# thetengda/OKVIS2-X

Hardware: AMD Instinct MI355X
Metric: Gauss-Newton iters/sec on 50-KF/2000-landmark window; ATE vs CPU ref (higher is better)
Workload: dtype f64; 1 GPU; 2048 independent S50 windows (50 KF / 2000 landmarks / 16000 reprojections, 49 IMU factors), DENSE_SCHUR + DOGLEG, all tolerances 0; windows_total=2048, windows_per_gpu=2048, parallelism=replicas x1 (one window batch per GPU, no collective in the loop)

## Files before the change

okvis2-x_amd/csrc/chol_tiles.hpp:

```cpp
#pragma once
#include "dev_clock.hpp"
#include "device_problem.hpp"
#include "okvisgpu_math.hpp"

namespace okg {

constexpr int kLd = kTile + 1;


typedef double dbl4 __attribute__((ext_vector_type(4)));

__device__ __forceinline__ bool cholSelect(const DevProblem& P, int w) {
  const WinState& s = P.st[w];
  return !s.done && s.need_gn && !s.gn_failed;
}

__device__ __forceinline__ int tileBlocks(const DevProblem& P, int w, int k) {
  const int fdim = P.win_fdim[w], g0 = P.win_sgap[2 * w], gl = P.win_sgap[2 * w + 1];
  int end = min(fdim - kTile * k, kTile);
  if (gl > 0 && g0 >= kTile * k && g0 < kTile * (k + 1)) end = min(end, g0 - kTile * k);
  return max(1, (end + 15) >> 4);
}

struct TileSrc {
  const double* S;
  const double* W;
  const int16_t* fu;
  int T;
  int64_t ld;
  __device__ __forceinline__ const double* at(int i, int j, int k) const {
    return (gmem(fu)[i * T + j] < k ? W : S) + (int64_t)i * kTile * ld + j * kTile;
  }
};
__device__ __forceinline__ TileSrc tileSrc(const DevProblem& P, int w, int64_t ld) {
  return TileSrc{P.S + P.win_soff[w], P.W + P.win_soff[w], P.tile_fu + P.win_tnzoff[w], (int)(ld / kTile), ld};
}

__device__ __forceinline__ void loadTile(const double* A, int64_t ld, int r0, int c0, double* s, int t) {
  double2 v[8];
#pragma unroll
  for (int u = 0; u < 8; ++u) {
    const int e = t + 256 * u, r = e >> 5, c = 2 * (e & 31);
    v[u] = *gmem(reinterpret_cast<const double2*>(A + (int64_t)(r0 + r) * ld + c0 + c));
  }
#pragma unroll
  for (int u = 0; u < 8; ++u) {
    const int e = t + 256 * u, r = e >> 5, c = 2 * (e & 31);
    s[r * kLd + c] = v[u].x;
    s[r * kLd + c + 1] = v[u].y;
  }
}

__device__ __forceinline__ void mfmaTileNT(const double* sA, const double* sB, dbl4 acc[2][2], int t) {
  const int wave = t >> 6, lane = t & 63;
  const int r0 = 32 * (wave >> 1), c0 = 32 * (wave & 1);
  const int lr = lane & 15, lk = lane >> 4;
#pragma unroll
  for (int a = 0; a < 2; ++a)
#pragma unroll
    for (int b = 0; b < 2; ++b) acc[a][b] = dbl4{0.0, 0.0, 0.0, 0.0};
#pragma unroll 4
  for (int kk = 0; kk < kTile; kk += 4) {
    double av[2], bv[2];
#pragma unroll
    for (int a = 0; a < 2; ++a) av[a] = sA[(r0 + 16 * a + lr) * kLd + kk + lk];
#pragma unroll
    for (int b = 0; b < 2; ++b) bv[b] = sB[(c0 + 16 * b + lr) * kLd + kk + lk];
#pragma unroll
    for (int a = 0; a < 2; ++a)
#pragma unroll
      for (int b = 0; b < 2; ++b) acc[a][b] = __builtin_amdgcn_mfma_f64_16x16x4f64(av[a], bv[b], acc[a][b], 0, 0, 0);
  }
}

template <bool SUB>
__device__ __forceinline__ void storeTile(double* A, int64_t ld, int r0g, int c0g, const dbl4 acc[2][2], int t) {
  const int wave = t >> 6, lane = t & 63;
  const int r0 = 32 * (wave >> 1), c0 = 32 * (wave & 1);
#pragma unroll
  for (int a = 0; a < 2; ++a)
#pragma unroll
    for (int b = 0; b < 2; ++b)
#pragma unroll
      for (int reg = 0; reg < 4; ++reg) {
        const int rr = r0 + 16 * a + (lane >> 4) + 4 * reg;
        const int cc = c0 + 16 * b + (lane & 15);
        auto dst = gmemw(A + (int64_t)(r0g + rr) * ld + c0g + cc);
        if (SUB) *dst -= acc[a][b][reg];
        else *dst = acc[a][b][reg];
      }
}

__device__ __forceinline__ void loadC(const double* A, int64_t ld, dbl4 c[2][2], int t) {
  const int wave = t >> 6, lane = t & 63;
  const int r0 = 32 * (wave >> 1), c0 = 32 * (wave & 1);
#pragma unroll
  for (int a = 0; a < 2; ++a)
#pragma unroll
    for (int b = 0; b < 2; ++b)
#pragma unroll
      for (int reg = 0; reg < 4; ++reg)
        c[a][b][reg] = gmem(A)[(int64_t)(r0 + 16 * a + (lane >> 4) + 4 * reg) * ld + c0 + 16 * b + (lane & 15)];
}
__device__ __forceinline__ void storeTileSub(double* A, int64_t ld, const dbl4 c[2][2], const dbl4 acc[2][2], int t) {
  const int wave = t >> 6, lane = t & 63;
  const int r0 = 32 * (wave >> 1), c0 = 32 * (wave & 1);
#pragma unroll
  for (int a = 0; a < 2; ++a)
#pragma unroll
    for (int b = 0; b < 2; ++b)
#pragma unroll
      for (int reg = 0; reg < 4; ++reg)
        gmemw(A)[(int64_t)(r0 + 16 * a + (lane >> 4) + 4 * reg) * ld + c0 + 16 * b + (lane & 15)] = c[a][b][reg] - acc[a][b][reg];
}

__device__ __forceinline__ double rsqrtRefined(double d) {
  double r = __builtin_amdgcn_rsq(d);
  const double h = 0.5 * d;
  r = r * (1.5 - h * r * r);
  r = r * (1.5 - h * r * r);
  return r;
}

template <int KB>
__device__ __forceinline__ void mfma16(const double* a, int lda, const double* b, int ldbk, int ldbn, double sign,
                                       dbl4& acc, int lane) {
  const int lr = lane & 15, lk = lane >> 4;
#pragma unroll
  for (int q = 0; q < 4 * KB; ++q) {
    const double av = sign * a[lr * lda + 4 * q + lk];
    const double bv = b[(4 * q + lk) * ldbk + lr * ldbn];
    acc = __builtin_amdgcn_mfma_f64_16x16x4f64(av, bv, acc, 0, 0, 0);
  }
}
__device__ __forceinline__ dbl4 loadC16(const double* c, int ldc, int lane) {
  dbl4 v;
#pragma unroll
  for (int r = 0; r < 4; ++r) v[r] = c[((lane >> 4) + 4 * r) * ldc + (lane & 15)];
  return v;
}
__device__ __forceinline__ void storeC16(double* c, int ldc, const dbl4& v, int lane) {
#pragma unroll
  for (int r = 0; r < 4; ++r) c[((lane >> 4) + 4 * r) * ldc + (lane & 15)] = v[r];
}

__device__ __forceinline__ int ldsAcquire(int* p) {
  return __hip_atomic_load(p, __ATOMIC_ACQUIRE, __HIP_MEMORY_SCOPE_WORKGROUP);
}
__device__ __forceinline__ void ldsRelease(int* p, int v) {
  __hip_atomic_store(p, v, __ATOMIC_RELEASE, __HIP_MEMORY_SCOPE_WORKGROUP);
}
__device__ __forceinline__ int ldsAcquireL(int* p) {
  const int v = __hip_atomic_load(p, __ATOMIC_RELAXED, __HIP_MEMORY_SCOPE_WORKGROUP);
  __builtin_amdgcn_fence(__ATOMIC_ACQUIRE, "workgroup", "local");
  return v;
}
__device__ __forceinline__ void ldsReleaseL(int* p, int v) {
  __builtin_amdgcn_fence(__ATOMIC_RELEASE, "workgroup", "local");
  __hip_atomic_store(p, v, __ATOMIC_RELAXED, __HIP_MEMORY_SCOPE_WORKGROUP);
}
#ifndef OKG_WAIT_SLEEP
#define OKG_WAIT_SLEEP 1
#endif
template <bool LOCAL = false>
__device__ __forceinline__ bool waitFlag(int* p, int v, int* fail) {
  for (;;) {
    if ((LOCAL ? ldsAcquireL(p) : ldsAcquire(p)) >= v) return true;
    if (LOCAL ? ldsAcquireL(fail) : ldsAcquire(fail)) return false;
    __builtin_amdgcn_s_sleep(OKG_WAIT_SLEEP);
  }
}
template <bool LOCAL = false>
__device__ __forceinline__ void waveBarrier(int* ctr, int& gen, int n, int lane) {
  ++gen;
  if (LOCAL) {
    __builtin_amdgcn_fence(__ATOMIC_RELEASE, "workgroup", "local");
    if (lane == 0) __hip_atomic_fetch_add(ctr, 1, __ATOMIC_RELAXED, __HIP_MEMORY_SCOPE_WORKGROUP);
    while (ldsAcquireL(ctr) < gen * n) __builtin_amdgcn_s_sleep(OKG_WAIT_SLEEP);
  } else {
    if (lane == 0) __hip_atomic_fetch_add(ctr, 1, __ATOMIC_RELEASE, __HIP_MEMORY_SCOPE_WORKGROUP);
    while (ldsAcquire(ctr) < gen * n) __builtin_amdgcn_s_sleep(OKG_WAIT_SLEEP);
  }
}

__device__ __forceinline__ bool chol8Row(const double* sA, int c0, double (&r)[8], double (&x)[8], double (&rl)[8]) {
  double D[8][8];
#pragma unroll
  for (int m = 0; m < 8; ++m)
#pragma unroll
    for (int k = 0; k <= m; ++k) D[m][k] = sA[(c0 + m) * kLd + c0 + k];
  bool bad = false;
#pragma unroll
  for (int c = 0; c < 8; ++c) {
    const double d = D[c][c];
    if (!(d > 0.0)) bad = true;
    rl[c] = rsqrtRefined(d);
#pragma unroll
    for (int m = c + 1; m < 8; ++m) D[m][c] *= rl[c];
    x[c] = r[c] * rl[c];
#pragma unroll
    for (int m = c + 1; m < 8; ++m) {
      D[m][m] -= D[m][c] * D[m][c];
      r[m] -= x[c] * D[m][c];
    }
#pragma unroll
    for (int m = c + 2; m < 8; ++m)
#pragma unroll
      for (int k = c + 1; k < m; ++k) D[m][k] -= D[m][c] * D[k][c];
  }
  return !bad;
}
__device__ __forceinline__ void storeRow8(double* sA, int c0, const double (&x)[8], int i) {
  if (i >= c0) {
#pragma unroll
    for (int k = 0; k < 8; ++k)
      if (i >= c0 + 8 || k <= i - c0) sA[i * kLd + c0 + k] = x[k];
  }
}
__device__ __forceinline__ void inv8(const double* sA, const double* sRl, double* xd, int c0, int lane) {
  if (lane >= 8) return;
  double L[8][8], rl[8];
#pragma unroll
  for (int m = 0; m < 8; ++m) {
    rl[m] = sRl[c0 + m];
#pragma unroll
    for (int k = 0; k < m; ++k) L[m][k] = sA[(c0 + m) * kLd + c0 + k];
  }
  double y[8];
#pragma unroll
  for (int m = 0; m < 8; ++m) {
    double v = (m == lane) ? 1.0 : 0.0;
#pragma unroll
    for (int k = 0; k < m; ++k) v -= L[m][k] * y[k];
    y[m] = v * rl[m];
  }
#pragma unroll
  for (int m = 0; m < 8; ++m) xd[m * kLd + lane] = y[m];
}
__device__ __forceinline__ bool subPanel8(double* sA, double* xd, double* sRl, int c0, int lane) {
  double r[8], x[8], rl[8];
#pragma unroll
  for (int k = 0; k < 8; ++k) r[k] = sA[lane * kLd + c0 + k];
  if (!chol8Row(sA, c0, r, x, rl)) return false;
  storeRow8(sA, c0, x, lane);
  if (lane == 0) {
#pragma unroll
    for (int k = 0; k < 8; ++k) sRl[c0 + k] = rl[k];
  }
  __builtin_amdgcn_wave_barrier();
  inv8(sA, sRl, xd, c0, lane);
  return true;
}

__device__ __forceinline__ void trailingFrom(double* sA, int c0, int cs, int wg, int nw, int lane) {
  const int cb0 = cs >> 4;
  const bool part = (cs & 15) != 0;
  const int lr = lane & 15, lk = lane >> 4;
  int idx = 0;
  for (int rb = cb0; rb < 4; ++rb)
    for (int cb = cb0; cb <= rb; ++cb, ++idx) {
      if (idx % nw != wg) continue;
      double* C = sA + 16 * rb * kLd + 16 * cb;
      dbl4 acc = loadC16(C, kLd, lane);
#pragma unroll
      for (int q = 0; q < 2; ++q) {
        const double av = -sA[(16 * rb + lr) * kLd + c0 + 4 * q + lk];
        const double bv = sA[(16 * cb + lr) * kLd + c0 + 4 * q + lk];
        acc = __builtin_amdgcn_mfma_f64_16x16x4f64(av, bv, acc, 0, 0, 0);
      }
      if (part && cb == cb0 && lr < 8) continue;
#pragma unroll
      for (int r = 0; r < 4; ++r)
        if (!(part && rb == cb0 && r < 2)) C[(lk + 4 * r) * kLd + lr] = acc[r];
    }
}
__device__ __forceinline__ void trailing8(double* sA, int c0, int wg, int nw, int lane) {
  trailingFrom(sA, c0, c0 + 8, wg, nw, lane);
}

__device__ __forceinline__ void xDiag16(const double* sA, double* sX, int q, int lane) {
  const int m = lane >> 3, j = lane & 7;
  const int b = 16 * q;
  double t = 0.0;
#pragma unroll
  for (int k = 0; k < 8; ++k) t += sA[(b + 8 + m) * kLd + b + k] * sX[(b + k) * kLd + b + j];
  sX[(b + 8 + m) * kLd + b + j] = t;
  __builtin_amdgcn_wave_barrier();
  double tk[8];
#pragma unroll
  for (int k = 0; k < 8; ++k) tk[k] = sX[(b + 8 + k) * kLd + b + j];
  double v = 0.0;
#pragma unroll
  for (int k = 0; k < 8; ++k) v += sX[(b + 8 + m) * kLd + b + 8 + k] * tk[k];
  __builtin_amdgcn_wave_barrier();
  sX[(b + 8 + m) * kLd + b + j] = -v;
}
__device__ __forceinline__ void xOffDiag16(const double* sA, double* sX, int q, int j, int lane) {
  dbl4 acc = dbl4{0.0, 0.0, 0.0, 0.0};
  for (int m = j; m < q; ++m)
    mfma16<1>(sA + 16 * q * kLd + 16 * m, kLd, sX + 16 * m * kLd + 16 * j, kLd, 1, 1.0, acc, lane);
  double* Xqj = sX + 16 * q * kLd + 16 * j;
  storeC16(Xqj, kLd, acc, lane);
  dbl4 x = dbl4{0.0, 0.0, 0.0, 0.0};
  mfma16<1>(sX + 16 * q * kLd + 16 * q, kLd, Xqj, kLd, 1, -1.0, x, lane);
  storeC16(Xqj, kLd, x, lane);
}
__device__ __forceinline__ void yBlock16(const double* sX, double* sy, int q, int lane) {
  const int r = 16 * q + (lane & 15), p = lane >> 4;
  double xv[16], rv[16];
#pragma unroll
  for (int it = 0; it < 16; ++it) {
    xv[it] = sX[r * kLd + p + 4 * it];
    rv[it] = sy[p + 4 * it];
  }
  double a = 0.0;
#pragma unroll
  for (int it = 0; it < 16; ++it) a += (p + 4 * it <= r) ? xv[it] * rv[it] : 0.0;
  a += __shfl_xor(a, 16, 64);
  a += __shfl_xor(a, 32, 64);
  if (p == 0) sy[kTile + r] = a;
}
__host__ __device__ constexpr bool persistentCaller(int kCaller) { return kCaller >= 10; }
template <int kCaller>
__device__ __forceinline__ void xStoreRows16(const double* sX, double* Li, int q, int g, int lane) {
  double2 v[3];
#pragma unroll
  for (int it = 0; it < 3; ++it) {
    const int e = min(64 * g + lane + 192 * it, 511), r = 16 * q + (e >> 5), c = 2 * (e & 31);
    v[it] = double2{(c <= r) ? sX[r * kLd + c] : 0.0, (c + 1 <= r) ? sX[r * kLd + c + 1] : 0.0};
  }
#pragma unroll
  for (int it = 0; it < 3; ++it) {
    const int e = 64 * g + lane + 192 * it, r = 16 * q + (e >> 5), c = 2 * (e & 31);
    if (e < 512 && (!persistentCaller(kCaller) || c <= r)) *gmemw(reinterpret_cast<double2*>(Li + r * kTile + c)) = v[it];
  }
}

__host__ __device__ constexpr bool teamCaller(int kCaller) { return kCaller >= 20; }
constexpr int kPotrfBarriers = 3;
template <int kCaller>
__device__ __forceinline__ void potrfSync(int* sFl, int& tgen, int lane) {
  if (teamCaller(kCaller)) waveBarrier<true>(&sFl[4], tgen, 4, lane);
  else ldsBarrier();
}
template <int kCaller>
__device__ __forceinline__ bool potrfTileBody(const double* Sg, int64_t ld, double* Li, double* workk, double* sA, double* sX,
                                              double* sy, double* sRl, int* sFl, int t, bool haveTile, int tgen0, int nq) {
  const int wave = t >> 6, lane = t & 63;
  int tgen = tgen0;
  CLK_INIT
  if (!haveTile) loadTile(Sg, ld, 0, 0, sA, t);
  nq = __builtin_amdgcn_readfirstlane(nq);
#pragma unroll
  for (int u = 0; u < 16; ++u) {
    const int e = t + 256 * u;
    sX[(e >> 6) * kLd + (e & 63)] = 0.0;
  }
  if (t < 4) sFl[t] = 0;
  potrfSync<kCaller>(sFl, tgen, lane);
  CLK(4)
  if (wave == 0) {
    const int i = lane;
    if (i >= 16 * nq) {
      sX[i * kLd + i] = 1.0;
      sy[kTile + i] = sy[i];
    }
    double xp[8];
#pragma unroll
    for (int k = 0; k < 8; ++k) xp[k] = 0.0;
#pragma unroll 1
    for (int s = 0; s < 2 * nq; ++s) {
      const int c0 = 8 * s;
      CLK(25)
      if (s >= 2 && !waitFlag<true>(&sFl[1], s - 1, &sFl[2])) break;
      CLK(21)
      double r[8], x[8], rl[8];
#pragma unroll
      for (int k = 0; k < 8; ++k) r[k] = sA[i * kLd + c0 + k];
      if (s >= 1) {
#pragma unroll
        for (int hb = 0; hb < 2; ++hb) {
          double Lq[4][8];
#pragma unroll
          for (int c = 0; c < 4; ++c)
#pragma unroll
            for (int m = 0; m < 8; ++m) Lq[c][m] = sA[(c0 + m) * kLd + c0 - 8 + 4 * hb + c];
#pragma unroll
          for (int c = 0; c < 4; ++c)
#pragma unroll
            for (int m = 0; m < 8; ++m) r[m] -= xp[4 * hb + c] * Lq[c][m];
        }
        asm volatile("" ::"v"(r[0]), "v"(r[1]), "v"(r[2]), "v"(r[3]), "v"(r[4]), "v"(r[5]), "v"(r[6]), "v"(r[7]));
        if (i >= c0) {
#pragma unroll
          for (int k = 0; k < 8; ++k) sA[i * kLd + c0 + k] = r[k];
        }
        __builtin_amdgcn_wave_barrier();
      }
      CLK(22)
      if (!chol8Row(sA, c0, r, x, rl)) {
        if (lane == 0) ldsReleaseL(&sFl[2], 1);
        break;
      }
      asm volatile("" ::"v"(x[7]));
      CLK(23)
      if (i >= c0) {
#pragma unroll
        for (int k = 0; k < 8; ++k) sA[i * kLd + c0 + k] = x[k];
      }
      if (lane == 0) {
#pragma unroll
        for (int k = 0; k < 8; ++k) sRl[c0 + k] = rl[k];
        ldsReleaseL(&sFl[0], s + 1);
      }
      CLK(24)
#pragma unroll
      for (int k = 0; k < 8; ++k) xp[k] = x[k];
    }
  } else {
    const int g = wave - 1;
    int gen = 0;
#pragma unroll 1
    for (int s = 0; s < 2 * nq; ++s) {
      if (!waitFlag<true>(&sFl[0], s + 1, &sFl[2])) break;
      if (g == 0) inv8(sA, sRl, sX + 8 * s * kLd + 8 * s, 8 * s, lane);
      if (s < 6) trailingFrom(sA, 8 * s, 8 * s + 16, g, 3, lane);
      waveBarrier<true>(&sFl[3], gen, 3, lane);
      if (g == 0 && lane == 0) ldsReleaseL(&sFl[1], s + 1);
      if (s & 1) {
        const int q = s >> 1;
        if (g == 0) xDiag16(sA, sX, q, lane);
        waveBarrier<true>(&sFl[3], gen, 3, lane);
        if (g < q) xOffDiag16(sA, sX, q, g, lane);
        waveBarrier<true>(&sFl[3], gen, 3, lane);
        if (g == 0) yBlock16(sX, sy, q, lane);
        for (int qs = q, qe = q + 1 < nq ? q + 1 : 4; qs < qe; ++qs) xStoreRows16<kCaller>(sX, Li, qs, g, lane);
      }
    }
  }
  potrfSync<kCaller>(sFl, tgen, lane);
  CLK(5)
  if (sFl[2]) return false;
  if (t < kTile) {
    const double y = sy[kTile + t];
    sy[t] = y;
    if (!persistentCaller(kCaller)) gmemw(workk)[t] = y;
  }
  potrfSync<kCaller>(sFl, tgen, lane);
  CLK(10)
  return true;
}
template <int kCaller>
__device__ __noinline__ bool potrfTile(const double* Sg, int64_t ld, double* Li, double* workk, double* sA, double* sX, double* sy,
                                      double* sRl, int* sFl, int t, bool haveTile, int tgen0 = 0, int nq = 4) {
  return potrfTileBody<kCaller>(Sg, ld, Li, workk, sA, sX, sy, sRl, sFl, t, haveTile, tgen0, nq);
}

__device__ __forceinline__ void accToLds(double* s, const dbl4 acc[2][2], int t) {
  const int wave = t >> 6, lane = t & 63;
  const int r0 = 32 * (wave >> 1), c0 = 32 * (wave & 1);
#pragma unroll
  for (int a = 0; a < 2; ++a)
#pragma unroll
    for (int b = 0; b < 2; ++b)
#pragma unroll
      for (int reg = 0; reg < 4; ++reg) s[(r0 + 16 * a + (lane >> 4) + 4 * reg) * kLd + c0 + 16 * b + (lane & 15)] = acc[a][b][reg];
}
__device__ __forceinline__ void accSubToLds(double* s, const dbl4 c[2][2], const dbl4 acc[2][2], int t) {
  const int wave = t >> 6, lane = t & 63;
  const int r0 = 32 * (wave >> 1), c0 = 32 * (wave & 1);
#pragma unroll
  for (int a = 0; a < 2; ++a)
#pragma unroll
    for (int b = 0; b < 2; ++b)
#pragma unroll
      for (int reg = 0; reg < 4; ++reg)
        s[(r0 + 16 * a + (lane >> 4) + 4 * reg) * kLd + c0 + 16 * b + (lane & 15)] = c[a][b][reg] - acc[a][b][reg];
}

__device__ __forceinline__ void mfmaPanelRows(const double* sA, const double* sX, dbl4 acc[4], int t) {
  const int wave = t >> 6, lane = t & 63;
  const int lr = lane & 15, lk = lane >> 4;
#pragma unroll
  for (int cb = 0; cb < 4; ++cb) acc[cb] = dbl4{0.0, 0.0, 0.0, 0.0};
#pragma unroll
  for (int kk = 0; kk < kTile; kk += 4) {
    const double av = sA[(16 * wave + lr) * kLd + kk + lk];
#pragma unroll
    for (int cb = kk >> 4; cb < 4; ++cb)
      acc[cb] = __builtin_amdgcn_mfma_f64_16x16x4f64(av, sX[(16 * cb + lr) * kLd + kk + lk], acc[cb], 0, 0, 0);
  }
}
__device__ __forceinline__ void storePanelRows(double* A, int64_t ld, const dbl4 acc[4], int t) {
  const int wave = t >> 6, lane = t & 63;
#pragma unroll
  for (int cb = 0; cb < 4; ++cb)
#pragma unroll
    for (int reg = 0; reg < 4; ++reg)
      gmemw(A)[(int64_t)(16 * wave + (lane >> 4) + 4 * reg) * ld + 16 * cb + (lane & 15)] = acc[cb][reg];
}
__device__ __forceinline__ void panelRowsToLds(double* s, const dbl4 acc[4], int t) {
  const int wave = t >> 6, lane = t & 63;
#pragma unroll
  for (int cb = 0; cb < 4; ++cb)
#pragma unroll
    for (int reg = 0; reg < 4; ++reg) s[(16 * wave + (lane >> 4) + 4 * reg) * kLd + 16 * cb + (lane & 15)] = acc[cb][reg];
}
__device__ __forceinline__ int diagRb(int wave, int e) { return wave == 0 ? (e == 0 ? 0 : 1) : (wave == 1 ? 2 : 3); }
__device__ __forceinline__ int diagCb(int wave, int e) { return wave == 0 ? (e == 0 ? 0 : e - 1) : (wave == 3 ? 2 + e : e); }
__device__ __forceinline__ int diagN(int wave) { return wave < 2 ? 3 : 2; }
__device__ __forceinline__ void mfmaDiagNT(const double* sL, dbl4 acc[3], int t) {
  const int wave = t >> 6, lane = t & 63;
  const int lr = lane & 15, lk = lane >> 4;
  const int n = diagN(wave);
  int ra[3], rb[3];
#pragma unroll
  for (int e = 0; e < 3; ++e) {
    ra[e] = (16 * diagRb(wave, e) + lr) * kLd + lk;
    rb[e] = (16 * diagCb(wave, e) + lr) * kLd + lk;
    acc[e] = dbl4{0.0, 0.0, 0.0, 0.0};
  }
#pragma unroll 4
  for (int kk = 0; kk < kTile; kk += 4) {
#pragma unroll
    for (int e = 0; e < 3; ++e)
      if (e < n) acc[e] = __builtin_amdgcn_mfma_f64_16x16x4f64(sL[ra[e] + kk], sL[rb[e] + kk], acc[e], 0, 0, 0);
  }
}
__device__ __forceinline__ int64_t diagAt(int wave, int e, int reg, int lane, int64_t ld) {
  return (int64_t)(16 * diagRb(wave, e) + (lane >> 4) + 4 * reg) * ld + 16 * diagCb(wave, e) + (lane & 15);
}
__device__ __forceinline__ void loadCDiag(const double* A, int64_t ld, dbl4 c[3], int t) {
  const int wave = t >> 6, lane = t & 63, n = diagN(wave);
#pragma unroll
  for (int e = 0; e < 3; ++e)
    if (e < n)
#pragma unroll
      for (int reg = 0; reg < 4; ++reg) c[e][reg] = gmem(A)[diagAt(wave, e, reg, lane, ld)];
}
__device__ __forceinline__ void storeDiagSub(double* A, int64_t ld, const dbl4 c[3], const dbl4 acc[3], int t) {
  const int wave = t >> 6, lane = t & 63, n = diagN(wave);
#pragma unroll
  for (int e = 0; e < 3; ++e)
    if (e < n)
#pragma unroll
      for (int reg = 0; reg < 4; ++reg) gmemw(A)[diagAt(wave, e, reg, lane, ld)] = c[e][reg] - acc[e][reg];
}
__device__ __forceinline__ void diagSubToLds(double* s, const dbl4 c[3], const dbl4 acc[3], int t) {
  const int wave = t >> 6, lane = t & 63, n = diagN(wave);
#pragma unroll
  for (int e = 0; e < 3; ++e)
    if (e < n)
#pragma unroll
      for (int reg = 0; reg < 4; ++reg) s[diagAt(wave, e, reg, lane, kLd)] = c[e][reg] - acc[e][reg];
}

struct WgSync {
  __device__ __forceinline__ void operator()() const { ldsBarrier(); }
};
template <class Sync = WgSync>
__device__ __forceinline__ void panelRhsVector(const double* sX, const double* sy, double* sz, double* sP, int t,
                                               Sync sync = Sync()) {
  const int c = t & 63, q = t >> 6;
  double a = 0.0;
#pragma unroll
  for (int r = 16 * q; r < 16 * q + 16; ++r) a += (r >= c) ? sX[r * kLd + c] * sy[r] : 0.0;
  sP[q * kTile + c] = a;
  sync();
  if (t < kTile) sz[t] = (sP[t] + sP[kTile + t]) + (sP[2 * kTile + t] + sP[3 * kTile + t]);
  sync();
}

__device__ __forceinline__ double panelRhsRow(const double* sA, const double* sz, int t) {
  const int row = t >> 2, q = t & 3;
  double a = 0.0;
#pragma unroll
  for (int c = 16 * q; c < 16 * q + 16; ++c) a += sA[row * kLd + c] * sz[c];
  a += __shfl_xor(a, 1, 64);
  a += __shfl_xor(a, 2, 64);
  return a;
}

template <class Sync = WgSync>
__device__ __forceinline__ void panelTile(const double* Aik, double* Lik, int64_t ld, double* worki, double* sA, const double* sX, const double* sz,
                          int t, double* defer = nullptr, Sync sync = Sync()) {
  loadTile(Aik, ld, 0, 0, sA, t);
  sync();
  dbl4 acc[4];
  mfmaPanelRows(sA, sX, acc, t);
  {
    const int row = t >> 2, q = t & 3;
    const double a = panelRhsRow(sA, sz, t);
    if (q == 0) {
      if (defer) defer[row] = a;
      else worki[row] -= a;
    }
  }
  sync();
  storePanelRows(Lik, ld, acc, t);
}


constexpr int kBsThreads = 1024;
constexpr int kBsPre = 3;
struct BsOps {
  double2 v[kBsPre][2];
  double2 li[2];
};
template <bool UPPER>
__device__ __forceinline__ const double* bsTile(const double* S, int64_t ld, int I, int i) {
  return UPPER ? S + (int64_t)I * kTile * ld + i * kTile : S + (int64_t)i * kTile * ld + I * kTile;
}
template <bool UPPER>
__device__ __forceinline__ void bsLoad(const double* S, int64_t ld, const double* Linv, const int* lst, int I, int vt,
                                       BsOps& o) {
  const int c2 = 2 * (vt & 31), rg = vt >> 5;
#ifdef OKG_BS_DUMMY_DIAG
  const int dummy = I;
#else
  const int dummy = lst[0] > 0 ? lst[1] : I;
#endif
#pragma unroll
  for (int m = 0; m < kBsPre; ++m) {
    const double* Lt = bsTile<UPPER>(S, ld, I, m < lst[0] ? lst[1 + m] : dummy) + c2;
#pragma unroll
    for (int u = 0; u < 2; ++u) o.v[m][u] = *gmem(reinterpret_cast<const double2*>(Lt + (int64_t)(rg + 32 * u) * ld));
  }
  const double* Li = Linv + (int64_t)I * kTile * kTile + c2;
#pragma unroll
  for (int u = 0; u < 2; ++u) o.li[u] = *gmem(reinterpret_cast<const double2*>(Li + (rg + 32 * u) * kTile));
}
__device__ __forceinline__ double sum32(const double* p) {
  double a[8];
#pragma unroll
  for (int k = 0; k < 8; ++k) a[k] = (p[kTile * k] + p[kTile * (k + 8)]) + (p[kTile * (k + 16)] + p[kTile * (k + 24)]);
  return ((a[0] + a[1]) + (a[2] + a[3])) + ((a[4] + a[5]) + (a[6] + a[7]));
}
template <bool UPPER>
__device__ __noinline__ double2 bsExtra(const double* S, int64_t ld, int T, const uint8_t* nz, int last, int I,
                                        const double* sx, int vt, double ax, double ay) {
  const int c2 = 2 * (vt & 31), rg = vt >> 5;
  for (int i = last + 1; i < T; ++i) {
    if (!nz[i * T + I]) continue;
    const double* Lt = bsTile<UPPER>(S, ld, I, i) + c2;
    const double* xi = sx + i * kTile + rg;
#pragma unroll
    for (int u = 0; u < 2; ++u) {
      const double2 v = *gmem(reinterpret_cast<const double2*>(Lt + (int64_t)(rg + 32 * u) * ld));
      ax += v.x * xi[32 * u];
      ay += v.y * xi[32 * u];
    }
  }
  return double2{ax, ay};
}
template <bool UPPER>
__device__ __forceinline__ void bsPartial(const double* S, int64_t ld, int T, const uint8_t* nz, const int* lst, int I,
                                          const BsOps& c, const double* sx, double* sA, int vt) {
  const int c2 = 2 * (vt & 31), rg = vt >> 5;
  double ax = 0.0, ay = 0.0;
#pragma unroll
  for (int m = 0; m < kBsPre; ++m) {
    const bool on = m < lst[0];
    const double* xi = sx + (on ? lst[1 + m] : I) * kTile + rg;
#pragma unroll
    for (int u = 0; u < 2; ++u) {
      ax += (on ? c.v[m][u].x : 0.0) * xi[32 * u];
      ay += (on ? c.v[m][u].y : 0.0) * xi[32 * u];
    }
  }
  if (lst[0] == kBsPre) {
    const double2 e = bsExtra<UPPER>(S, ld, T, nz, lst[kBsPre], I, sx, vt, ax, ay);
    ax = e.x;
    ay = e.y;
  }
  sA[rg * kTile + c2] = ax;
  sA[rg * kTile + c2 + 1] = ay;
}
__device__ __forceinline__ void bsDiag(const BsOps& c, const double* sy, double* sA, int vt) {
  const int c2 = 2 * (vt & 31), rg = vt >> 5;
  double bx = 0.0, by = 0.0;
#pragma unroll
  for (int u = 0; u < 2; ++u) {
    const int r = rg + 32 * u;
    bx += (r >= c2) ? c.li[u].x * sy[r] : 0.0;
    by += (r >= c2 + 1) ? c.li[u].y * sy[r] : 0.0;
  }
  sA[rg * kTile + c2] = bx;
  sA[rg * kTile + c2 + 1] = by;
}
__device__ __forceinline__ void bsList(const uint8_t* nz, int T, int I, int* lst) {
  int n = 0;
  for (int i = I + 1; i < T && n < kBsPre; ++i)
    if (nz[i * T + I]) lst[1 + n++] = i;
  lst[0] = n;
}
__device__ __forceinline__ void gnFinalizeRow(const DevProblem& P, size_t i, double x) {
  const double dg = gmem(P.diagF)[i], sc = gmem(P.sF)[i], g = gmem(P.gF)[i];
  P.yF[i] = x;
  P.gnF[i] = -dg * x;
  const double gr = sc * g / dg;
  P.dgF[i] = gr;
  P.vF[i] = gr / dg;
}
__device__ __forceinline__ bool gapRow(const DevProblem& P, int w, int e) {
  const int g0 = P.win_sgap[2 * w];
  return e >= g0 && e < g0 + P.win_sgap[2 * w + 1];
}

template <int NT = 256>
__device__ __forceinline__ void backSubstitute(const DevProblem& P, int w, const double* S, int64_t ld, int T, const double* Linv,
                               const uint8_t* nz, double* sx, double* sA, double* sy, int t) {
  const auto sync = [] { __syncthreads(); };
  sync();
  constexpr int kV = kBsThreads / NT;
  for (int I = T - 1; I >= 0; --I) {
    int lst[1 + kBsPre];
    bsList(nz, T, I, lst);
    BsOps c[kV];
#pragma unroll
    for (int k = 0; k < kV; ++k) bsLoad<false>(S, ld, Linv, lst, I, t + NT * k, c[k]);
#pragma unroll
    for (int k = 0; k < kV; ++k) bsPartial<false>(S, ld, T, nz, lst, I, c[k], sx, sA, t + NT * k);
    sync();
    if (t < kTile) sy[t] = sx[I * kTile + t] - sum32(sA + t);
    sync();
#pragma unroll
    for (int k = 0; k < kV; ++k) bsDiag(c[k], sy, sA, t + NT * k);
    sync();
    if (t < kTile) sx[I * kTile + t] = sum32(sA + t);
    sync();
  }
  const int fdim = P.win_fdim[w];
  for (int e = t; e < fdim; e += NT)
    if (!gapRow(P, w, e)) gnFinalizeRow(P, (size_t)P.win_foff[w] + e, sx[e]);
}

}
```

okvis2-x_amd/csrc/kernels_chol.hip:

```cpp
#include "chol_tiles.hpp"
#include "launch.hpp"

namespace okg {

#ifndef OKG_CHOL_OCC
#define OKG_CHOL_OCC 2
#endif

template <int MODE>
__global__ __launch_bounds__(256, OKG_CHOL_OCC) void k_cholesky(const DevProblem* __restrict__ Pp) {
  const DevProblem& P = *Pp;
  const int w = MODE == 1 ? (int)(blockIdx.x >> 1) : (int)blockIdx.x, part = MODE == 1 ? (int)(blockIdx.x & 1) : 0;
  if (!cholSelect(P, w)) return;
  const int64_t ld = P.win_fpad[w];
  const int T = (int)(ld / kTile);
  const int tL = MODE == 0 ? 0 : P.win_bsplit[2 * w], tS = MODE == 0 ? 0 : P.win_bsplit[2 * w + 1];
  const bool split = MODE != 0 && tS > 0;
  if ((MODE == 1 && part == 1 && !split) || (MODE == 2 && !split)) return;
  const int k0 = !split ? 0 : (MODE == 2 ? tS : (part == 0 ? 0 : tL));
  const int k1 = !split ? T : (MODE == 2 ? T : (part == 0 ? tL : tS));
  const int jEnd = split && MODE == 1 && part == 1 ? tS : T;
  const bool finish = !split || MODE == 2;
  const TileSrc cur = tileSrc(P, w, ld);
  double* W = P.W + P.win_soff[w];
  double* Linv = P.Linv + P.win_linvoff[w];
  const uint8_t* nz = P.tile_nz + P.win_tnzoff[w];
  double* work = P.fwdF + P.win_fwdoff[w];
  double* defer = split ? P.chol_defer + P.win_defoff[w] : nullptr;
  __shared__ double sA[kTile * kLd];
  __shared__ double sX[kTile * kLd];
  __shared__ double sy[2 * kTile];
  __shared__ double sRl[kTile];
  __shared__ int sFl[4];
  const int t = threadIdx.x;
  const int fdim = P.win_fdim[w];
  CLK_INIT
  extern __shared__ double sxDyn[];
  if (MODE == 2) {
    for (int e = t; e < ld; e += 256) sxDyn[e] = work[e];
  } else {
    for (int e = t; e < ld; e += 256) sxDyn[e] = (e < fdim) ? P.rhsF[(size_t)P.win_foff[w] + e] : 0.0;
  }
  __syncthreads();
  int tStep = t;
  auto bandUpdate = [&](int k, int jLo, bool toLds) {
    const int t = tStep;
    int xHeld = -1;
    bool inLds = false;
    for (int i = T - 1; i > k && i >= jLo; --i) {
      if (!nz[i * T + k]) continue;
      const bool aInX = xHeld == i;
      const double* aBuf = aInX ? sX : sA;
      bool aLoaded = aInX;
      for (int j = max(k + 1, jLo); j <= i && j < jEnd; ++j) {
        if (!nz[j * T + k]) continue;
        if (!aLoaded) {
          loadTile(W + i * kTile * ld + k * kTile, ld, 0, 0, sA, t);
          aLoaded = true;
        }
        const double* bBuf = aBuf;
        if (j != i) {
          if (aInX) {
            loadTile(W + j * kTile * ld + k * kTile, ld, 0, 0, sA, t);
            bBuf = sA;
          } else {
            if (xHeld != j) loadTile(W + j * kTile * ld + k * kTile, ld, 0, 0, sX, t);
            xHeld = j;
            bBuf = sX;
          }
        }
        ldsBarrier();
        double* Cij = W + i * kTile * ld + j * kTile;
        if (j == i) {
          dbl4 c[3], acc[3];
          loadCDiag(cur.at(i, j, k), ld, c, t);
          mfmaDiagNT(aBuf, acc, t);
          if (toLds && i == k + 1) {
            ldsBarrier();
            diagSubToLds(sA, c, acc, t);
            inLds = true;
          } else {
            storeDiagSub(Cij, ld, c, acc, t);
          }
        } else {
          dbl4 c[2][2], acc[2][2];
          loadC(cur.at(i, j, k), ld, c, t);
          mfmaTileNT(aBuf, bBuf, acc, t);
          storeTileSub(Cij, ld, c, acc, t);
        }
        ldsBarrier();
      }
    }
    return inLds;
  };
  if (MODE == 2) {
    for (int k = tL; k < tS; ++k) {
      for (int i = tS; i < T; ++i)
        if (nz[i * T + k] && t < kTile)
          sxDyn[i * kTile + t] -= defer[((size_t)(i - tS) * (tS - tL) + (k - tL)) * kTile + t];
      __syncthreads();
      bandUpdate(k, tS, false);
      __syncthreads();
    }
  }
  bool haveDiag = false;
  for (int k = k0; k < k1; ++k) {
    CLK(11)
    if (t < kTile) sy[t] = sxDyn[k * kTile + t];
    __syncthreads();
    if (!potrfTile<10 + MODE>(cur.at(k, k, k), ld, Linv + (int64_t)k * kTile * kTile, nullptr, sA, sX,
                   sy, sRl, sFl, t, haveDiag, 0, tileBlocks(P, w, k))) {
      if (t == 0) P.st[w].gn_failed = 1;
      return;
    }
    if (t < kTile) sxDyn[k * kTile + t] = sy[t];
    CLK(0)
    tStep = t;
    asm volatile("" : "+v"(tStep));
    panelRhsVector(sX, sy, sy + kTile, sA, t);
    for (int i = k + 1; i < T; ++i)
      if (nz[i * T + k])
        panelTile(cur.at(i, k, k), W + i * kTile * ld + k * kTile, ld, sxDyn + i * kTile, sA, sX, sy + kTile, tStep,
                  i >= jEnd ? defer + ((size_t)(i - tS) * (tS - tL) + (k - tL)) * kTile : nullptr);
    __syncthreads();
    CLK(1)
    haveDiag = bandUpdate(k, 0, true);
  }
  CLK(2)
  if (!finish) {
    const int e0 = part == 0 ? 0 : tL * kTile, e1 = part == 0 ? tL * kTile : tS * kTile;
    for (int e = t; e < ld; e += 256)
      if ((e >= e0 && e < e1) || (part == 0 && e >= tS * kTile)) work[e] = sxDyn[e];
    return;
  }
  backSubstitute(P, w, W, ld, T, Linv, nz, sxDyn, sA, sy, t);
  CLK(3)
  CHOL_CLK_REPORT(T)
}

__global__ __launch_bounds__(256, 2) void k_chol_roots(const DevProblem* __restrict__ Pp) {
  const DevProblem& P = *Pp;
  const int w = P.chol_root_items[3 * blockIdx.x], d = P.chol_root_items[3 * blockIdx.x + 1];
  const bool first = P.chol_root_items[3 * blockIdx.x + 2] != 0;
  if (!cholSelect(P, w)) return;
  const int64_t ld = P.win_fpad[w];
  const int T = (int)(ld / kTile);
  const TileSrc cur = tileSrc(P, w, ld);
  double* work = P.fwdF + P.win_fwdoff[w];
  const uint8_t* nz = P.tile_nz + P.win_tnzoff[w];
  __shared__ double sA[kTile * kLd];
  __shared__ double sX[kTile * kLd];
  __shared__ double sy[2 * kTile];
  __shared__ double sRl[kTile];
  __shared__ int sFl[4];
  const int t = threadIdx.x;
  const int fdim = P.win_fdim[w];
  const double* rhs = P.rhsF + P.win_foff[w];
  for (int e = t; e < ld; e += 256) {
    const int b = e / kTile;
    bool mine = b == d;
    if (first && b != d) {
      bool root = true;
      for (int q = 0; q < b && root; ++q) root = !nz[b * T + q];
      mine = !root;
    }
    if (mine) work[e] = e < fdim ? rhs[e] : 0.0;
  }
  __syncthreads();
  if (t < kTile) sy[t] = work[d * kTile + t];
  __syncthreads();
  if (!potrfTile<1>(cur.at(d, d, d), ld, P.Linv + P.win_linvoff[w] + (int64_t)d * kTile * kTile,
                    work + d * kTile, sA, sX, sy, sRl, sFl, t, false, 0, tileBlocks(P, w, d)))
    if (t == 0) P.st[w].gn_failed = 1;
}


__global__ __launch_bounds__(256, 2) void k_chol_update(const DevProblem* __restrict__ Pp, int launch) {
  const DevProblem& P = *Pp;
  const int item = P.chol_upd_begin[launch] + blockIdx.x;
  const int4 it = reinterpret_cast<const int4*>(P.chol_upd_items)[item];
  const int w = it.x, i = it.y, j = it.z, mode = it.w & 0xff, k = it.w >> 8;
  if (!cholSelect(P, w)) return;
  const int64_t ld = P.win_fpad[w];
  const TileSrc cur = tileSrc(P, w, ld);
  double* W = P.W + P.win_soff[w];
  double* work = P.fwdF + P.win_fwdoff[w];
  __shared__ double sA[kTile * kLd];
  __shared__ double sX[kTile * kLd];
  __shared__ double sB[kTile * kLd];
  __shared__ double sy[2 * kTile];
  __shared__ double sRl[kTile];
  __shared__ int sFl[4];
  const int t = threadIdx.x;
  {
    loadTile(P.Linv + P.win_linvoff[w] + (int64_t)k * kTile * kTile, kTile, 0, 0, sX, t);
    loadTile(cur.at(i, k, k), ld, 0, 0, sA, t);
    if (j != i) loadTile(cur.at(j, k, k), ld, 0, 0, sB, t);
    if (i == j && t < kTile) sy[t] = work[k * kTile + t];
    const int row = t >> 2, q = t & 3;
    const double rhsOld = (i == j && q == 0) ? work[i * kTile + row] : 0.0;
    __syncthreads();
    if (i == j) panelRhsVector(sX, sy, sy + kTile, sB, t);
    dbl4 li[4], lj[4];
    mfmaPanelRows(sA, sX, li, t);
    if (j != i) mfmaPanelRows(sB, sX, lj, t);
    if (i == j) {
      const double a = panelRhsRow(sA, sy + kTile, t);
      if (q == 0) {
        const double nr = rhsOld - a;
        gmemw(work)[i * kTile + row] = nr;
        if (mode & 2) sRl[row] = nr;
      }
    }
    ldsBarrier();
    panelRowsToLds(sA, li, t);
    if (j != i) panelRowsToLds(sB, lj, t);
    double* Cij = W + i * kTile * ld + j * kTile;
    if (i == j) {
      dbl4 c[3];
      loadCDiag(cur.at(i, j, k), ld, c, t);
      storePanelRows(W + k * kTile * ld + i * kTile, ld, li, t);
      ldsBarrier();
      dbl4 acc[3];
      mfmaDiagNT(sA, acc, t);
      if (mode & 2) {
        ldsBarrier();
        diagSubToLds(sA, c, acc, t);
        __syncthreads();
        if (t < kTile) sy[t] = sRl[t];
      } else {
        storeDiagSub(Cij, ld, c, acc, t);
      }
    } else {
      dbl4 c[2][2];
      loadC(cur.at(i, j, k), ld, c, t);
      ldsBarrier();
      dbl4 acc[2][2];
      mfmaTileNT(sA, sB, acc, t);
      storeTileSub(Cij, ld, c, acc, t);
    }
  }
  if (!(mode & 2)) return;
  const int d = i;
  __syncthreads();
  if (!potrfTile<2>(cur.at(d, d, d), ld, P.Linv + P.win_linvoff[w] + (int64_t)d * kTile * kTile,
                    work + d * kTile, sA, sX, sy, sRl, sFl, t, true, 0, tileBlocks(P, w, d)))
    if (t == 0) P.st[w].gn_failed = 1;
}

constexpr int kBsReal = 512;
__global__ __launch_bounds__(kBsReal) void k_chol_bsub(const DevProblem* __restrict__ Pp) {
  constexpr int kV = kBsThreads / kBsReal;
  const DevProblem& P = *Pp;
  const int w = blockIdx.x, h = blockIdx.y;
  if (!cholSelect(P, w)) return;
  const int64_t ld = P.win_fpad[w];
  const int T = (int)(ld / kTile);
  const int tL = P.win_bsplit[2 * w], tS = P.win_bsplit[2 * w + 1];
  const bool split = tS > 0;
  if (h == 1 && !split) return;
  const int nSep = split ? T - tS : T;
  const int nSteps = nSep + (split ? (h == 0 ? tL : tS - tL) : 0);
  const int partTop = h == 0 ? tL - 1 : tS - 1;
  auto rowAt = [&](int n) { return n < nSep ? T - 1 - n : partTop - (n - nSep); };
  const double* S = P.W + P.win_soff[w];
  const double* work = P.fwdF + P.win_fwdoff[w];
  const double* Linv = P.Linv + P.win_linvoff[w];
  __shared__ double sA[32 * kTile];
  __shared__ double sy[kTile];
  extern __shared__ double sx[];
  int* lists = reinterpret_cast<int*>(sx + ld);
  uint8_t* nz = reinterpret_cast<uint8_t*>(lists + (1 + kBsPre) * T);
  const int t = threadIdx.x;
  CLK_INIT
  for (int e = t; e < T * T; e += kBsReal) nz[e] = P.tile_nz[P.win_tnzoff[w] + e];
  for (int e = t; e < ld; e += kBsReal) sx[e] = work[e];
  if (t < T) bsList(P.tile_nz + P.win_tnzoff[w], T, t, lists + (1 + kBsPre) * t);
  __syncthreads();
  BsOps ping[kV], pong[kV];
  auto load = [&](int I, BsOps* o) {
#pragma unroll
    for (int k = 0; k < kV; ++k) bsLoad<true>(S, ld, Linv, lists + (1 + kBsPre) * I, I, t + kBsReal * k, o[k]);
  };
  auto step = [&](int I, const BsOps* c) {
    const int* lst = lists + (1 + kBsPre) * I;
#pragma unroll
    for (int k = 0; k < kV; ++k) bsPartial<true>(S, ld, T, nz, lst, I, c[k], sx, sA, t + kBsReal * k);
    ldsBarrier();
    if (t < kTile) sy[t] = sx[I * kTile + t] - sum32(sA + t);
    ldsBarrier();
#pragma unroll
    for (int k = 0; k < kV; ++k) bsDiag(c[k], sy, sA, t + kBsReal * k);
    ldsBarrier();
    if (t < kTile) sx[I * kTile + t] = sum32(sA + t);
    ldsBarrier();
  };
  load(rowAt(0), ping);
  CLK(12)
  for (int n = 0; n < nSteps; n += 2) {
    load(rowAt(min(n + 1, nSteps - 1)), pong);
    step(rowAt(n), ping);
    if (n + 1 == nSteps) break;
    load(rowAt(min(n + 2, nSteps - 1)), ping);
    step(rowAt(n + 1), pong);
  }
  CLK(13)
  const int fdim = P.win_fdim[w];
  const int e0 = !split ? 0 : (h == 0 ? 0 : tL * kTile), e1 = !split ? fdim : (h == 0 ? fdim : tS * kTile);
  for (int e = e0 + t; e < e1; e += kBsReal)
    if ((!split || h == 1 || e < tL * kTile || e >= tS * kTile) && !gapRow(P, w, e))
      gnFinalizeRow(P, (size_t)P.win_foff[w] + e, sx[e]);
  BSUB_CLK_REPORT(T)
}

void launch_cholesky_split_b(const DevProblem& P, hipStream_t s) {
  hipLaunchKernelGGL(k_cholesky<2>, dim3(P.n_win), dim3(256), sizeof(double) * P.max_fpad, s, P.self);
}

size_t cholesky_persistent_lds() {
  hipFuncAttributes attr;
  if (hipFuncGetAttributes(&attr, reinterpret_cast<const void*>(k_cholesky<0>)) != hipSuccess) return ~size_t(0) >> 1;
  return attr.sharedSizeBytes;
}

void launch_cholesky(const DevProblem& P, hipStream_t s) {
  if (P.n_win == 0) return;
  if (P.chol_schedule == 4 || P.chol_schedule == 5) {
    launch_cholesky_pipe(P, s, P.chol_schedule == 5);
    return;
  }
  if (P.chol_schedule == 1) {
    hipLaunchKernelGGL(k_cholesky<0>, dim3(P.n_win), dim3(256), sizeof(double) * P.max_fpad, s, P.self);
    return;
  }
  if (P.chol_schedule == 3) {
    hipLaunchKernelGGL(k_cholesky<1>, dim3(2 * P.n_win), dim3(256), sizeof(double) * P.max_fpad, s, P.self);
    hipLaunchKernelGGL(k_cholesky<2>, dim3(P.n_win), dim3(256), sizeof(double) * P.max_fpad, s, P.self);
    return;
  }
  hipLaunchKernelGGL(k_chol_roots, dim3(P.n_chol_roots), dim3(256), 0, s, P.self);
  for (int l = 1; l < P.n_chol_launches; ++l) {
    const int nu = P.h_upd_begin[l + 1] - P.h_upd_begin[l];
    if (nu > 0) hipLaunchKernelGGL(k_chol_update, dim3(nu), dim3(256), 0, s, P.self, l);
  }
  hipLaunchKernelGGL(k_chol_bsub, dim3(P.n_win, 2), dim3(kBsReal),
                     sizeof(double) * P.max_fpad + sizeof(int) * (1 + kBsPre) * P.max_tiles + P.max_tiles * P.max_tiles, s,
                     P.self);
}

}
```

Before: 218,900 window-iterations/s.

## Hand panel tiles from registers to LDS for trailing update

Panel tile results computed in registers are kept (up to three most recent) and written straight into LDS buffers. The following band update then reuses them instead of reloading those tiles from global memory. For three panel tiles an explicit six-step update schedule is used. This removes global reloads of freshly stored panel tiles, at the cost of extra live registers (three dbl4[4] sets), which may cut occupancy, and more complex synchronisation logic.

```diff
diff --git a/okvis2-x_amd/csrc/chol_tiles.hpp b/okvis2-x_amd/csrc/chol_tiles.hpp
--- a/okvis2-x_amd/csrc/chol_tiles.hpp
+++ b/okvis2-x_amd/csrc/chol_tiles.hpp
@@ -582,11 +582,10 @@
 }
 
 template <class Sync = WgSync>
-__device__ __forceinline__ void panelTile(const double* Aik, double* Lik, int64_t ld, double* worki, double* sA, const double* sX, const double* sz,
-                          int t, double* defer = nullptr, Sync sync = Sync()) {
+__device__ __forceinline__ void panelTileKeep(const double* Aik, double* Lik, int64_t ld, double* worki, double* sA, const double* sX,
+                                              const double* sz, dbl4 acc[4], int t, double* defer = nullptr, Sync sync = Sync()) {
   loadTile(Aik, ld, 0, 0, sA, t);
   sync();
-  dbl4 acc[4];
   mfmaPanelRows(sA, sX, acc, t);
   {
     const int row = t >> 2, q = t & 3;
@@ -598,6 +597,12 @@
   }
   sync();
   storePanelRows(Lik, ld, acc, t);
+}
+template <class Sync = WgSync>
+__device__ __forceinline__ void panelTile(const double* Aik, double* Lik, int64_t ld, double* worki, double* sA, const double* sX, const double* sz,
+                          int t, double* defer = nullptr, Sync sync = Sync()) {
+  dbl4 acc[4];
+  panelTileKeep(Aik, Lik, ld, worki, sA, sX, sz, acc, t, defer, sync);
 }
 
 
diff --git a/okvis2-x_amd/csrc/kernels_chol.hip b/okvis2-x_amd/csrc/kernels_chol.hip
--- a/okvis2-x_amd/csrc/kernels_chol.hip
+++ b/okvis2-x_amd/csrc/kernels_chol.hip
@@ -6,6 +6,17 @@
 #ifndef OKG_CHOL_OCC
 #define OKG_CHOL_OCC 2
 #endif
+#ifndef OKG_CHOL_HANDOVER
+#define OKG_CHOL_HANDOVER 1
+#endif
+#ifndef OKG_CHOL_HOLD2
+#define OKG_CHOL_HOLD2 1
+#endif
+#ifndef OKG_CHOL_HANDOVER_LDSBAR
+#define OKG_CHOL_HANDOVER_LDSBAR 0
+#endif
+
+struct PersistSync : WgSync {};
 
 template <int MODE>
 __global__ __launch_bounds__(256, OKG_CHOL_OCC) void k_cholesky(const DevProblem* __restrict__ Pp) {
@@ -43,25 +54,50 @@
   }
   __syncthreads();
   int tStep = t;
-  auto bandUpdate = [&](int k, int jLo, bool toLds) {
+  auto updTile = [&](int k, int i, int j, const double* aBuf, const double* bBuf, bool toLds) __attribute__((always_inline)) {
     const int t = tStep;
-    int xHeld = -1;
+    bool inLds = false;
+    ldsBarrier();
+    double* Cij = W + i * kTile * ld + j * kTile;
+    if (j == i) {
+      dbl4 c[3], acc[3];
+      loadCDiag(cur.at(i, j, k), ld, c, t);
+      mfmaDiagNT(aBuf, acc, t);
+      if (toLds && i == k + 1) {
+        ldsBarrier();
+        diagSubToLds(sA, c, acc, t);
+        inLds = true;
+      } else {
+        storeDiagSub(Cij, ld, c, acc, t);
+      }
+    } else {
+      dbl4 c[2][2], acc[2][2];
+      loadC(cur.at(i, j, k), ld, c, t);
+      mfmaTileNT(aBuf, bBuf, acc, t);
+      storeTileSub(Cij, ld, c, acc, t);
+    }
+    ldsBarrier();
+    return inLds;
+  };
+  auto bandUpdate = [&](int k, int jLo, bool toLds, int aHeld, int xHeld) __attribute__((always_inline)) {
+    const int t = tStep;
     bool inLds = false;
     for (int i = T - 1; i > k && i >= jLo; --i) {
       if (!nz[i * T + k]) continue;
       const bool aInX = xHeld == i;
       const double* aBuf = aInX ? sX : sA;
-      bool aLoaded = aInX;
+      if (!OKG_CHOL_HANDOVER) aHeld = -1;
       for (int j = max(k + 1, jLo); j <= i && j < jEnd; ++j) {
         if (!nz[j * T + k]) continue;
-        if (!aLoaded) {
+        if (!aInX && aHeld != i) {
           loadTile(W + i * kTile * ld + k * kTile, ld, 0, 0, sA, t);
-          aLoaded = true;
+          aHeld = i;
         }
         const double* bBuf = aBuf;
         if (j != i) {
           if (aInX) {
-            loadTile(W + j * kTile * ld + k * kTile, ld, 0, 0, sA, t);
+            if (!OKG_CHOL_HANDOVER || aHeld != j) loadTile(W + j * kTile * ld + k * kTile, ld, 0, 0, sA, t);
+            aHeld = j;
             bBuf = sA;
           } else {
             if (xHeld != j) loadTile(W + j * kTile * ld + k * kTile, ld, 0, 0, sX, t);
@@ -69,26 +105,7 @@
             bBuf = sX;
           }
         }
-        ldsBarrier();
-        double* Cij = W + i * kTile * ld + j * kTile;
-        if (j == i) {
-          dbl4 c[3], acc[3];
-          loadCDiag(cur.at(i, j, k), ld, c, t);
-          mfmaDiagNT(aBuf, acc, t);
-          if (toLds && i == k + 1) {
-            ldsBarrier();
-            diagSubToLds(sA, c, acc, t);
-            inLds = true;
-          } else {
-            storeDiagSub(Cij, ld, c, acc, t);
-          }
-        } else {
-          dbl4 c[2][2], acc[2][2];
-          loadC(cur.at(i, j, k), ld, c, t);
-          mfmaTileNT(aBuf, bBuf, acc, t);
-          storeTileSub(Cij, ld, c, acc, t);
-        }
-        ldsBarrier();
+        inLds |= updTile(k, i, j, aBuf, bBuf, toLds);
       }
     }
     return inLds;
@@ -99,7 +116,7 @@
         if (nz[i * T + k] && t < kTile)
           sxDyn[i * kTile + t] -= defer[((size_t)(i - tS) * (tS - tL) + (k - tL)) * kTile + t];
       __syncthreads();
-      bandUpdate(k, tS, false);
+      bandUpdate(k, tS, false, -1, -1);
       __syncthreads();
     }
   }
@@ -117,14 +134,48 @@
     CLK(0)
     tStep = t;
     asm volatile("" : "+v"(tStep));
-    panelRhsVector(sX, sy, sy + kTile, sA, t);
-    for (int i = k + 1; i < T; ++i)
-      if (nz[i * T + k])
-        panelTile(cur.at(i, k, k), W + i * kTile * ld + k * kTile, ld, sxDyn + i * kTile, sA, sX, sy + kTile, tStep,
-                  i >= jEnd ? defer + ((size_t)(i - tS) * (tS - tL) + (k - tL)) * kTile : nullptr);
-    __syncthreads();
+    panelRhsVector(sX, sy, sy + kTile, sA, tStep, PersistSync());
+    dbl4 h0[4], h1[4], h2[4];
+#pragma unroll
+    for (int c = 0; c < 4; ++c) h0[c] = h1[c] = h2[c] = dbl4{0.0, 0.0, 0.0, 0.0};
+    int np = 0, q0 = -1, q1 = -1, q2 = -1;
+    for (int i = k + 1; i < T; ++i) {
+      if (!nz[i * T + k]) continue;
+      if (OKG_CHOL_HANDOVER) {
+#pragma unroll
+        for (int c = 0; c < 4; ++c) {
+          h2[c] = h1[c];
+          h1[c] = h0[c];
+        }
+        q2 = q1;
+        q1 = q0;
+        q0 = i;
+      }
+      ++np;
+      panelTileKeep(cur.at(i, k, k), W + i * kTile * ld + k * kTile, ld, sxDyn + i * kTile, sA, sX, sy + kTile, h0, tStep,
+                    i >= jEnd ? defer + ((size_t)(i - tS) * (tS - tL) + (k - tL)) * kTile : nullptr);
+    }
+    if (OKG_CHOL_HANDOVER && np >= 1) panelRowsToLds(sA, h0, tStep);
+    if (OKG_CHOL_HANDOVER && (np == 2 || np == 3)) panelRowsToLds(sX, h1, tStep);
+    if (!(OKG_CHOL_HANDOVER && OKG_CHOL_HANDOVER_LDSBAR) || np == 0 || np > 3 || (np == 3 && !OKG_CHOL_HOLD2)) __syncthreads();
     CLK(1)
-    haveDiag = bandUpdate(k, 0, true);
+    if (!(OKG_CHOL_HANDOVER && np == 3)) {
+      haveDiag = bandUpdate(k, 0, true, q0, np == 2 ? q1 : -1);
+    } else {
+      haveDiag = false;
+#pragma unroll 1
+      for (int s = 0; s < 6; ++s) {
+        const int i = s == 2 || s == 4 ? q1 : (s == 5 ? q2 : q0);
+        const int j = s == 0 ? q0 : (s <= 2 ? q1 : q2);
+        if (j >= jEnd) continue;
+        if (s == 3) panelRowsToLds(sX, h2, tStep);
+        if (s == 4) {
+          if (OKG_CHOL_HOLD2) panelRowsToLds(sA, h1, tStep);
+          else loadTile(W + q1 * kTile * ld + k * kTile, ld, 0, 0, sA, tStep);
+        }
+        haveDiag |= updTile(k, i, j, s == 2 || s == 5 ? sX : sA, s == 0 ? sA : sX, true);
+      }
+    }
   }
   CLK(2)
   if (!finish) {
```

Result: no change. 220,500 window-iterations/s (median of 6 runs) (+0.7%).
